# yifangao112/DinoUNet

Hardware: AMD Instinct MI355X
Metric: 2D slices/sec training, dinounet_l 512x512 bf16 (higher is better)
Workload: dtype bf16; 1 GPU; dinounet_l train step (fwd+loss+bwd+clip+SGD), 512x512x3 slices, batch 8/GPU, frozen ViT + adapter + FAPM + U-Net decoder, random-init weights; global_batch=8, parallelism=dp1

## Files before the change

dinounet_amd/_build.py:

```python
import hashlib
import os
import subprocess
import sys

HERE = os.path.dirname(os.path.abspath(__file__))
CSRC = os.path.join(HERE, "csrc")
LIB = os.path.join(HERE, "libdinounet_hip.so")
SOURCES = ["gemm.hip", "gemm_bf16.hip", "gemm_glds.hip", "gemm_p8.hip", "gemm_rk.hip", "gemm_skinny.hip", "conv_halo.hip", "conv_strip.hip", "attention.hip", "norm.hip", "msda.hip", "elementwise.hip", "loss.hip", "optim.hip", "augment.hip", "export.hip", "surface.hip"]
FLAGS = ["--offload-arch=gfx950", "-O3", "-std=c++17", "-fPIC", "-munsafe-fp-atomics", "-fno-gpu-rdc"]
if os.environ.get("DINOUNET_DEBUG_KNOBS") == "1":
    FLAGS.append("-DDU_DEBUG_KNOBS")
EXTRA_FLAGS = {"attention.hip": ["-mllvm", "-amdgpu-mfma-vgpr-form"], "conv_strip.hip": ["-mllvm", "-amdgpu-mfma-vgpr-form"]}
NO_SCRATCH = ("gemm_bf16.hip", "gemm_glds.hip", "gemm_p8.hip", "gemm_rk.hip", "gemm_skinny.hip", "conv_halo.hip", "conv_strip.hip", "attention.hip", "surface.hip")
REMARK = "-Rpass-analysis=kernel-resource-usage"
import re as _re
_ABLATION = _re.compile(
    r"attn_fwd_kernelILi\d+ELb1EEE"
    r"|attn_fwd_w64_kernelILi\d+ELi\d+ELb1E"
    r"|attn_fwd_w64_kernelILi\d+ELi\d+ELb\dELi\d+ELi[1-9]\d*ELi\d+EEE"
    r"|attn_fwd_pipe_kernelILb1ELi\d+EEE|attn_fwd_pipe_kernelILb\dELi[1-9]\d*EEE")


def _digest():
    h = hashlib.sha256()
    for f in sorted(os.listdir(CSRC)) + ["../../include/dinounet_hip.h"]:
        p = os.path.join(CSRC, f)
        if os.path.isfile(p):
            h.update(f.encode())
            h.update(open(p, "rb").read())
    h.update(" ".join(FLAGS).encode())
    h.update(repr(sorted(EXTRA_FLAGS.items())).encode())
    return h.hexdigest()


def build(force: bool = False, verbose: bool = True) -> str:
    stamp = LIB + ".stamp"
    dig = _digest()
    if not force and os.path.exists(LIB) and os.path.exists(stamp) and open(stamp).read() == dig:
        return LIB
    hipcc = os.environ.get("HIPCC", "/opt/rocm/bin/hipcc")
    objs, procs = [], []
    os.makedirs(os.path.join(HERE, "build"), exist_ok=True)
    for s in SOURCES:
        o = os.path.join(HERE, "build", s.replace(".hip", ".o"))
        objs.append(o)
        cmd = [hipcc, *FLAGS, *EXTRA_FLAGS.get(s, []), *([REMARK] if s in NO_SCRATCH else []), "-c", os.path.join(CSRC, s), "-o", o]
# ... 31 lines not shown
```

dinounet_amd/csrc/elementwise.hip:

```cpp
#include <stdlib.h>
#include "common.h"

namespace {

__host__ int grid_1d(long total) {
  long g = (total + 255) / 256;
  if (g < 1) g = 1;
  if (g > 65535L * 8) g = 65535L * 8;
  return (int)g;
}

#define GRID_STRIDE(i, total) for (long i = (long)blockIdx.x * 256 + threadIdx.x; i < (total); i += (long)gridDim.x * 256)

struct PyrPix { int b, s0, Hs, Ws, yo, xo; };
__device__ __forceinline__ PyrPix pyr_decode(long p, int H, int W) {
  const int n = (H * W) >> 2, N = 21 * n;
  PyrPix q;
  q.b = (int)(p / N);
  int t = (int)(p - (long)q.b * N);
  if (t < 16 * n) { q.s0 = 0; q.Hs = 2 * H; q.Ws = 2 * W; }
  else if (t < 20 * n) { q.s0 = 16 * n; q.Hs = H; q.Ws = W; t -= 16 * n; }
  else { q.s0 = 20 * n; q.Hs = H >> 1; q.Ws = W >> 1; t -= 20 * n; }
  q.yo = t / q.Ws; q.xo = t - q.yo * q.Ws;
  return q;
// ... 1065 lines not shown

extern "C" int du_patchify16(int dst_dtype, const float* src, void* dst, int B, int C, int H, int W, void* stream) {
  hipStream_t st = (hipStream_t)stream;
  if (!src || !dst || B <= 0 || H % 16 || W % 16) return DU_ERR_BAD_ARG;
  long total = (long)B * (H / 16) * (W / 16) * C * 256;
  DISPATCH_T(dst_dtype,
             hipLaunchKernelGGL(patchify16_kernel<bf16_t>, dim3(grid_1d(total)), dim3(256), 0, st, src, (bf16_t*)dst, B, C, H, W, total),
             hipLaunchKernelGGL(patchify16_kernel<float>, dim3(grid_1d(total)), dim3(256), 0, st, src, (float*)dst, B, C, H, W, total));
  return du_check_launch();
}

extern "C" int du_msda_prep(int dtype, const void* raw, int64_t ldr, const float* ref, float* loc, float* attn, int64_t rows, int Lq,
                            int M, int P, int Hs, int Ws, void* stream) {
  hipStream_t st = (hipStream_t)stream;
  if (!raw || !ref || !loc || !attn || rows <= 0 || Lq <= 0 || rows % Lq || M <= 0 || P <= 0 || P > 16) return DU_ERR_BAD_ARG;
  long total = rows * M;
  DISPATCH_T(dtype,
             hipLaunchKernelGGL(msda_prep_kernel<bf16_t>, dim3(grid_1d(total)), dim3(256), 0, st, (const bf16_t*)raw, ldr, ref, loc, attn, (long)rows, Lq, M, P, 1.f / Ws, 1.f / Hs, total),
             hipLaunchKernelGGL(msda_prep_kernel<float>, dim3(grid_1d(total)), dim3(256), 0, st, (const float*)raw, ldr, ref, loc, attn, (long)rows, Lq, M, P, 1.f / Ws, 1.f / Hs, total));
  return du_check_launch();
}

extern "C" int du_msda_prep_bwd(int dtype, const float* attn, const float* gloc, const float* gattn, void* graw, int64_t ldr, int64_t rows,
                                int M, int P, int Hs, int Ws, void* stream) {
  hipStream_t st = (hipStream_t)stream;
  if (!attn || !gloc || !gattn || !graw || rows <= 0 || M <= 0 || P <= 0) return DU_ERR_BAD_ARG;
  long total = rows * M;
  DISPATCH_T(dtype,
             hipLaunchKernelGGL(msda_prep_bwd_kernel<bf16_t>, dim3(grid_1d(total)), dim3(256), 0, st, attn, gloc, gattn, (bf16_t*)graw, ldr, (long)rows, M, P, 1.f / Ws, 1.f / Hs, total),
             hipLaunchKernelGGL(msda_prep_bwd_kernel<float>, dim3(grid_1d(total)), dim3(256), 0, st, attn, gloc, gattn, (float*)graw, ldr, (long)rows, M, P, 1.f / Ws, 1.f / Hs, total));
  return du_check_launch();
}

extern "C" int du_act_bwd(int dtype, const void* z, const void* dy, void* dz, int64_t n, int act, void* stream) {
  hipStream_t st = (hipStream_t)stream;
  if (!z || !dy || !dz || n <= 0) return DU_ERR_BAD_ARG;
  DISPATCH_T(dtype,
             hipLaunchKernelGGL(act_bwd_kernel<bf16_t>, dim3(grid_1d(n)), dim3(256), 0, st, (const bf16_t*)z, (const bf16_t*)dy, (bf16_t*)dz, (long)n, act),
             hipLaunchKernelGGL(act_bwd_kernel<float>, dim3(grid_1d(n)), dim3(256), 0, st, (const float*)z, (const float*)dy, (float*)dz, (long)n, act));
  return du_check_launch();
}

extern "C" int du_se_gate_fwd(const float* sums, float inv_count, const float* W1, const float* b1, const float* W2, const float* b2,
                              float* hidden, float* gate, int B, int C, int R, void* stream) {
  hipStream_t st = (hipStream_t)stream;
  if (!sums || !W1 || !b1 || !W2 || !b2 || !hidden || !gate || B <= 0 || C <= 0 || R <= 0) return DU_ERR_BAD_ARG;
  hipLaunchKernelGGL(se_gate_fwd_kernel, dim3(B), dim3(256), (C + R) * sizeof(float), st, sums, inv_count, W1, b1, W2, b2, hidden, gate, C, R);
  return du_check_launch();
}

extern "C" int du_se_scale_fwd(int dtype, const void* x, int64_t ldx, const float* gate, const void* shortcut, int64_t ldsc, void* y,
                               int64_t ldy, int B, int64_t P, int C, void* stream) {
  hipStream_t st = (hipStream_t)stream;
  const int v = dtype == DU_BF16 ? 8 : 4;
  if (!x || !gate || !y || B <= 0 || P <= 0 || C % v || ldx % v || ldy % v || (shortcut && ldsc % v)) return DU_ERR_BAD_ARG;
  long total = (long)B * P * (C / v);
  DISPATCH_T(dtype,
             hipLaunchKernelGGL(se_scale_kernel<bf16_t>, dim3(grid_1d(total)), dim3(256), 0, st, (const bf16_t*)x, ldx, gate, (const bf16_t*)shortcut, ldsc, (bf16_t*)y, ldy, (long)P, C, total),
             hipLaunchKernelGGL(se_scale_kernel<float>, dim3(grid_1d(total)), dim3(256), 0, st, (const float*)x, ldx, gate, (const float*)shortcut, ldsc, (float*)y, ldy, (long)P, C, total));
  return du_check_launch();
}

extern "C" int du_se_gate_bwd(const float* dsum, const float* sums, float inv_count, const float* gate, const float* hidden,
                              const float* W1, const float* W2, float* dpool, float* dW1, float* db1, float* dW2, float* db2, int B, int C,
                              int R, void* stream) {
  hipStream_t st = (hipStream_t)stream;
  if (!dsum || !sums || !gate || !hidden || !W1 || !W2 || !dpool || !dW1 || !db1 || !dW2 || !db2 || B <= 0 || C <= 0 || R <= 0)
    return DU_ERR_BAD_ARG;
  int Bc = (int)(8000 / (long)(C + R));
  if (Bc < 1) return DU_ERR_UNSUPPORTED;
  if (Bc > B) Bc = B;
  hipLaunchKernelGGL(se_gate_bwd_kernel, dim3(1), dim3(1024), (size_t)2 * Bc * (C + R) * sizeof(float), st, dsum, sums, inv_count, gate, hidden,
// ... 339 lines not shown
```

dinounet_amd/csrc/gemm_p8.hip:

```cpp
#include <algorithm>
#include <vector>
#include "common.h"
#include "gemm_params.h"
#include "gemm_plan.h"
#include "gemm_skinny_body.h"

namespace {

typedef __attribute__((address_space(3))) void lds_void;

constexpr int PBM = 256, PBN = 256, PBK = 64;
constexpr int HALF_B = 128 * PBK * 2;
constexpr int BUF_B = 4 * HALF_B;
constexpr int STG_LD = PBN + 4;

template <typename TC> struct Out4p;
template <> struct Out4p<float> {
  static __device__ __forceinline__ void load(const float* p, float* v) { float4 t = *(const float4*)p; v[0] = t.x; v[1] = t.y; v[2] = t.z; v[3] = t.w; }
  static __device__ __forceinline__ void store(float* p, const float* v) { *(float4*)p = make_float4(v[0], v[1], v[2], v[3]); }
};
template <> struct Out4p<bf16_t> {
  static __device__ __forceinline__ void load(const bf16_t* p, float* v) {
    bf16x4 t = __builtin_bit_cast(bf16x4, *(const uint2*)p);
#pragma unroll
// ... 2020 lines not shown
    attr_set[g_p8_sched ? 1 : 0] = true;
  }
  hipLaunchKernelGGL(kfn, grid, dim3(512), P8_LDS, st, P);
  return du_check_launch();
}

int g_p8_tn = 1;

template <int SCHED, bool GA>
int launch_p8_tn(const du_gemm_args& a, int splits, hipStream_t st) {
  GemmParams P = make_params(a, DU_PLAIN_COL, GA ? DU_IM2COL_COL : DU_PLAIN_COL, PBM, PBN, PBK);
  P.tiles_m = (a.M + PBM - 1) / PBM;
  P.split_k = splits;
  P.k_per_split = 0;
  P.dbg = g_p8_debug;
  dim3 grid(P.tiles_m * P.tiles_n * splits, 1);
  void (*kfn)(GemmParams) = GA ? gemm_nt_p8_kernel<float, SCHED, true, true> : gemm_nt_p8_kernel<float, SCHED, true, false>;
  static bool attr_set = false;
  if (!attr_set) {
    if (hipFuncSetAttribute((const void*)kfn, hipFuncAttributeMaxDynamicSharedMemorySize, P8_LDS) != hipSuccess) return DU_ERR_LAUNCH;
    attr_set = true;
  }
  hipLaunchKernelGGL(kfn, grid, dim3(512), P8_LDS, st, P);
  return du_check_launch();
}

}

extern int g_attn_w;
extern int g_attn_impl, g_attn_thresh_log2, g_attn_var;
extern int g_rk_mode;
extern int g_wgrad_rows;
extern int g_ln_rows2;

extern "C" int du_set_option(int key, int value) {
  switch (key) {
    case 4: g_attn_w = value; return DU_OK;
    case 6: g_attn_impl = value; return DU_OK;
    case 7: g_attn_thresh_log2 = value; return DU_OK;
    case 8: g_attn_var = value; return DU_OK;
    case 0: g_p8_mode = value; return DU_OK;
    case 1: g_p8_sched = value; return DU_OK;
    case 2: g_p8_group = value; return DU_OK;
    case 3: g_p8_debug = value; return DU_OK;
    case 5: g_p8_tn = value; return DU_OK;
    case 9: g_p8_corun = value < 1 ? 1 : (value > 8 ? 8 : value); return DU_OK;
    case 10: g_p8_persist = value; return DU_OK;
    case 11: g_p8_pp_full = value; return DU_OK;
    case 12: g_rk_mode = value; return DU_OK;
    case 13: g_wgrad_rows = value; return DU_OK;
    case 14: g_p8_res = value; return DU_OK;
    case 15: g_p8_tail_inline = value; return DU_OK;
    case 16: g_p8_ks = value; return DU_OK;
    case 17: g_p8_tail_slices = value; return DU_OK;
    case 18: g_ln_rows2 = value; return DU_OK;
    default: return DU_ERR_BAD_ARG;
  }
}

static bool convt_gather_geom(const du_gemm_args& a, const void* src, long ld, long pixels_in) {
  const du_conv_geom& g = a.geom;
  if (g.KH != 2 || g.KW != 2 || g.stride != 2 || g.pad != 0 || g.transposed || g.p2) return false;
  if (g.Hi != 2 * g.Ho || g.Wi != 2 * g.Wo || g.Ho <= 0 || g.Wo <= 0) return false;
  if (g.C <= 0 || (g.C & (g.C - 1)) || g.C % 64 || ld % 8 || (((uintptr_t)src) & 15)) return false;
  if (pixels_in % ((long)g.Ho * g.Wo)) return false;
  return 4 * pixels_in * ld * 2 <= 0x7fffffffL;
}
static bool p8_gather_legal(const du_gemm_args& a) {
  if (a.a_mode != DU_IM2COL_ROW || a.b_mode != DU_PLAIN_ROW || a.dtype != DU_BF16 || a.out_dtype != DU_BF16) return false;
  if (a.split_k > 1 || a.batch > 1 || a.store_mode != DU_STORE_PLAIN || a.act == DU_ACT_SWIGLU) return false;
  if (!convt_gather_geom(a, a.A, a.lda, a.M) || a.K != 4 * a.geom.C) return false;
  if (a.K % 128 || a.M < 256 || a.N < 128 || a.N % 4 || a.ldb % 8 || (((uintptr_t)a.B) & 15)) return false;
  return (long)a.ldb * 2 * 256 <= 0x7fffffffL;
}

bool p8_legal(const du_gemm_args& a) {
  if (a.a_mode != DU_PLAIN_ROW || a.b_mode != DU_PLAIN_ROW || a.dtype != DU_BF16) return false;
  if (a.split_k > 1) return false;
  if (a.store_mode == DU_STORE_MSDA_PREP) {
    if (a.out_dtype != DU_F32 || a.residual || a.gamma || a.row_scale || a.alpha != 1.0f || a.act != DU_ACT_NONE || a.batch > 1) return false;
    if (a.N % 12 || a.N > 256 || a.ps_H <= 0 || a.ps_W <= 0 || a.ps_C <= 0 || !a.rope_sin || !a.C2) return false;
    if ((((uintptr_t)a.C) | ((uintptr_t)a.C2)) & 15) return false;
  } else
  if (a.store_mode == DU_STORE_QKV_ROPE || a.store_mode == DU_STORE_QKV_HEADS) {
    if (a.out_dtype != DU_BF16 || a.residual || a.gamma || a.row_scale || a.alpha != 1.0f || a.act != DU_ACT_NONE || a.batch > 1) return false;
    if (a.ps_H <= 0 || a.ps_W < a.ps_H || a.ps_C <= 0 || a.N != 3 * a.ps_C * 64 || a.ldc % 8 || (((uintptr_t)a.C) & 15)) return false;
    if (a.store_mode == DU_STORE_QKV_ROPE && (!a.rope_sin || !a.rope_cos || ((((uintptr_t)a.rope_sin) | ((uintptr_t)a.rope_cos)) & 15))) return false;
  } else
// ... 242 lines not shown
```

dinounet_amd/ops.py:

```python
import ctypes as C
import math
import os
import weakref

import torch

from . import _lib
from ._lib import (ACT_GELU, ACT_LEAKY, ACT_NONE, ACT_RELU, ACT_SWIGLU, DU_BF16, DU_F32, IM2COL_COL, IM2COL_ROW, PLAIN_COL,
                   PLAIN_ROW, STORE_MSDA_PREP, STORE_PIXEL_SHUFFLE2, STORE_QKV_HEADS, STORE_QKV_ROPE, STORE_SLABS, ConvGeom, GemmArgs)

__all__ = ["mm", "linear", "conv2d", "conv_transpose2x2", "norm_act", "layer_norm", "msda", "dwconv3x3",
           "maxpool3x3s2", "bilinear_add", "bilinear_resize", "squeeze_excite", "dice_ce_loss", "dice_ce_masked_loss", "dice_bce_loss",
           "labels_to_regions", "val_dice_ce", "val_dice_bce"]


def _code(dt):
    if dt == torch.bfloat16:
        return DU_BF16
    if dt == torch.float32:
        return DU_F32
    raise RuntimeError(f"dinounet_amd: unsupported dtype {dt} (bf16 / fp32 only)")


def _req(*ts):
# ... 1713 lines not shown
        ctx.lc_saved = None
        ctx.save_for_backward(xs, wq, attn)
        ctx.prep = (M, P, Hs, Ws, ncol)
        return loc, attn

    @staticmethod
    def backward(ctx, gloc, gattn):
        x, wq, attn = ctx.saved_tensors
        M, P, Hs, Ws, ncol = ctx.prep
        rows = attn.shape[0]
        graw = torch.empty((rows, ncol), dtype=x.dtype, device=attn.device)
        _lib.check(_lib.lib().du_msda_prep_bwd(_code(x.dtype), _p(attn), _p(gloc.contiguous()), _p(gattn.contiguous()), _p(graw), ncol, rows,
                                               M, P, Hs, Ws, _st()), "du_msda_prep_bwd")
        return (*_linear_cat_bwd(ctx, graw, x, wq), None, None, None, None, None, None)


def offsets_prep(x, w1, w2, b1, b2, ref, Lq, M, P, Hs, Ws):
    return _OffsetsPrep.apply(x.reshape(-1, x.shape[-1]), w1, w2, b1, b2, ref, Lq, M, P, Hs, Ws)


class _DWConvSegs(torch.autograd.Function):

    @staticmethod
    def forward(ctx, x, w, bias, segs, act):
        x = x.contiguous()
        Cc = w.shape[0]
        wf = _f32(w).view(Cc, 9)
        bf = _f32(bias)
        y = torch.empty_like(x)
        z = torch.empty_like(x) if act != ACT_NONE else None
        es = x.element_size()
        L = _lib.lib()
        for (off, B, h, ww, ld, bs) in segs:
            _lib.check(L.du_dwconv3x3_fwd(_code(x.dtype), C.c_void_p(x.data_ptr() + off * es), ld, bs, _p(wf), _p(bf),
                                          C.c_void_p(y.data_ptr() + off * es), ld, bs,
                                          None if z is None else C.c_void_p(z.data_ptr() + off * es), B, h, ww, Cc, act, _st()),
                       "du_dwconv3x3_fwd")
        ctx.save_for_backward(x, wf, z)
        ctx.conf = (segs, act, bias is not None, Cc)
        return y

    @staticmethod
    def backward(ctx, dy):
        x, wf, z = ctx.saved_tensors
        segs, act, has_bias, Cc = ctx.conf
        L = _lib.lib()
        es = x.element_size()
        code = _code(x.dtype)
        dy = dy.contiguous()
        if act != ACT_NONE:
            dz = torch.empty_like(dy)
            _lib.check(L.du_act_bwd(code, _p(z), _p(dy), _p(dz), dy.numel(), act, _st()), "du_act_bwd")
        else:
            dz = dy
        dx = torch.empty_like(x)
        dw = torch.empty((Cc, 9), dtype=torch.float32, device=x.device)
        db = torch.empty(Cc, dtype=torch.float32, device=x.device) if has_bias else None
        for si, (off, B, h, ww, ld, bs) in enumerate(segs):
            _lib.check(L.du_dwconv3x3_bwd_data(code, C.c_void_p(dz.data_ptr() + off * es), ld, bs, _p(wf),
                                               C.c_void_p(dx.data_ptr() + off * es), ld, bs, B, h, ww, Cc, _st()),
                       "du_dwconv3x3_bwd_data")
            n = int(L.du_dwconv_wgrad_ws_elems(code, B, h, ww, Cc))
            ws = torch.empty(max(n, 1), dtype=torch.float32, device=x.device)
            _lib.check(L.du_dwconv3x3_bwd_weight(code, C.c_void_p(x.data_ptr() + off * es), ld, bs,
                                                 C.c_void_p(dz.data_ptr() + off * es), ld, bs, _p(dw), _p(db), B, h, ww, Cc,
                                                 _p(ws), n, 1 if si > 0 else 0, _st()), "du_dwconv3x3_bwd_weight")
        return dx, dw.view(Cc, 1, 3, 3), db, None, None


def dwconv3x3(x, w, bias=None, act=ACT_NONE):
    x = x.contiguous()
    B, H, W, Cc = x.shape
    return _DWConvSegs.apply(x, w, bias, ((0, B, H, W, Cc, H * W * Cc),), act)


class _DWConvTokens(torch.autograd.Function):

    @staticmethod
    def forward(ctx, x, w, bias, H, W, act):
        x = x.contiguous()
        B, N, Cc = x.shape
        wf = _f32(w).view(Cc, 9)
        y = torch.empty_like(x)
        z = torch.empty_like(x) if act != ACT_NONE else None
        _lib.check(_lib.lib().du_dwconv3x3_tokens_fwd(_code(x.dtype), _p(x), _p(wf), _p(_f32(bias)), _p(y), _p(z), B, H, W, Cc, act, _st()),
                   "du_dwconv3x3_tokens_fwd")
        ctx.save_for_backward(x, wf, z)
        ctx.conf = (H, W, act, bias is not None)
        return y

    @staticmethod
    def backward(ctx, dy):
        x, wf, z = ctx.saved_tensors
        H, W, act, has_bias = ctx.conf
        B, N, Cc = x.shape
        L = _lib.lib()
        code = _code(x.dtype)
        dy = dy.contiguous()
        if act != ACT_NONE:
            dz = torch.empty_like(dy)
            _lib.check(L.du_act_bwd(code, _p(z), _p(dy), _p(dz), dy.numel(), act, _st()), "du_act_bwd")
        else:
            dz = dy
        dx = torch.empty_like(x)
        _lib.check(L.du_dwconv3x3_tokens_bwd_data(code, _p(dz), _p(wf), _p(dx), B, H, W, Cc, _st()), "du_dwconv3x3_tokens_bwd_data")
        dw = torch.empty((Cc, 9), dtype=torch.float32, device=x.device)
        db = torch.empty(Cc, dtype=torch.float32, device=x.device) if has_bias else None
        n = int(L.du_dwconv_wgrad_ws_elems(code, B, N, 1, Cc))
        ws = torch.empty(max(n, 1), dtype=torch.float32, device=x.device)
        _lib.check(L.du_dwconv3x3_tokens_bwd_weight(code, _p(x), _p(dz), _p(dw), _p(db), B, H, W, Cc, _p(ws), n, _st()),
                   "du_dwconv3x3_tokens_bwd_weight")
        return dx, dw.view(Cc, 1, 3, 3), db, None, None, None


def dwconv_tokens(x, w, bias, H, W, act=ACT_GELU):
    B, N, Cc = x.shape
    assert N == 21 * ((H * W) // 4) and H % 2 == 0 and W % 2 == 0, (N, H, W)
    return _DWConvTokens.apply(x, w, bias, H, W, act)


class _MaxPool(torch.autograd.Function):
    @staticmethod
    def forward(ctx, x):
        x = x.contiguous()
        B, H, W, Cc = x.shape
        Ho, Wo = (H - 1) // 2 + 1, (W - 1) // 2 + 1
        y = torch.empty((B, Ho, Wo, Cc), dtype=x.dtype, device=x.device)
        idx = torch.empty((B, Ho, Wo, Cc), dtype=torch.uint8, device=x.device)
        _lib.check(_lib.lib().du_maxpool3x3s2_fwd(_code(x.dtype), _p(x), _p(y), _p(idx), B, H, W, Cc, _st()), "du_maxpool3x3s2_fwd")
        ctx.save_for_backward(idx)
        ctx.shape = (B, H, W, Cc, x.dtype)
# ... 533 lines not shown
```

include/dinounet_hip.h:

```cpp
#ifndef DINOUNET_HIP_H
#define DINOUNET_HIP_H

#include <stdint.h>

#ifdef __cplusplus
extern "C" {
#endif

#define DU_OK 0
#define DU_ERR_BAD_ARG (-1)
#define DU_ERR_UNSUPPORTED (-2)
#define DU_ERR_LAUNCH (-3)

#define DU_F32 0
#define DU_BF16 1

#define DU_PLAIN_ROW 0
#define DU_PLAIN_COL 1
#define DU_IM2COL_ROW 2
#define DU_IM2COL_COL 3

#define DU_ACT_NONE 0
#define DU_ACT_GELU 1
#define DU_ACT_RELU 2
// ... 125 lines not shown
                     const float* sampling_loc, const float* attn_weight, const void* grad_out, float* grad_value,
                     float* grad_sampling_loc, float* grad_attn_weight, int N, int S, int M, int D, int L, int Lq, int P,
                     float* ws, int64_t ws_elems, void* stream);

int du_msda_forward_f64(const double* value, const int64_t* spatial_shapes, const int64_t* level_start_index, const double* sampling_loc,
                        const double* attn_weight, double* out, int N, int S, int M, int D, int L, int Lq, int P, void* stream);
int du_msda_backward_f64(const double* value, const int64_t* spatial_shapes, const int64_t* level_start_index, const double* sampling_loc,
                         const double* attn_weight, const double* grad_out, double* grad_value, double* grad_sampling_loc,
                         double* grad_attn_weight, int N, int S, int M, int D, int L, int Lq, int P, void* stream);

int du_msda_backward_bf16gv(const void* value, const int64_t* spatial_shapes, const int64_t* level_start_index, const float* sampling_loc,
                            const float* attn_weight, const void* grad_out, void* grad_value_bf16, float* grad_sampling_loc,
                            float* grad_attn_weight, int N, int S, int M, int D, int L, int Lq, int P, float* ws, int64_t ws_elems,
                            void* stream);

int du_msda_prep(int dtype, const void* raw, int64_t ldr, const float* ref, float* loc, float* attn, int64_t rows, int Lq,
                 int M, int P, int Hs, int Ws, void* stream);
int du_msda_prep_bwd(int dtype, const float* attn, const float* gloc, const float* gattn, void* graw, int64_t ldr,
                     int64_t rows, int M, int P, int Hs, int Ws, void* stream);

int du_dwconv3x3_fwd(int dtype, const void* x, int64_t ldx, int64_t xbs, const float* w, const float* bias, void* y,
                     int64_t ldy, int64_t ybs, void* z, int B, int H, int W, int C, int act, void* stream);
int du_dwconv3x3_bwd_data(int dtype, const void* dy, int64_t lddy, int64_t dybs, const float* w, void* dx, int64_t lddx,
                          int64_t dxbs, int B, int H, int W, int C, void* stream);
int64_t du_dwconv_wgrad_ws_elems(int dtype, int B, int H, int W, int C);
int du_dwconv3x3_bwd_weight(int dtype, const void* x, int64_t ldx, int64_t xbs, const void* dy, int64_t lddy, int64_t dybs,
                            float* dw, float* db, int B, int H, int W, int C, float* ws, int64_t ws_elems, int accumulate,
                            void* stream);
int du_dwconv3x3_tokens_fwd(int dtype, const void* x, const float* w, const float* bias, void* y, void* z, int B, int H, int W, int C,
                            int act, void* stream);
int du_dwconv3x3_tokens_bwd_data(int dtype, const void* dy, const float* w, void* dx, int B, int H, int W, int C, void* stream);
int du_dwconv3x3_tokens_bwd_weight(int dtype, const void* x, const void* dy, float* dw, float* db, int B, int H, int W, int C, float* ws,
                                   int64_t ws_elems, void* stream);
int du_maxpool3x3s2_fwd(int dtype, const void* x, void* y, uint8_t* idx, int B, int H, int W, int C, void* stream);
int du_maxpool3x3s2_bwd(int dtype, const uint8_t* idx, const void* dy, void* dx, int B, int H, int W, int C, void* stream);
int du_bilinear_add_fwd(int src_dtype, int dtype, const void* src, int64_t lds_, const void* base, int64_t ldb, void* out,
                        int64_t ldo, int B, int Hs, int Ws, int Ho, int Wo, int C, void* stream);
int du_bilinear_resize_bwd(int dtype, const void* dy, int64_t lddy, void* dx, int64_t lddx, int B, int Hs, int Ws, int Ho, int Wo,
                           int C, void* stream);
int du_act_bwd(int dtype, const void* z, const void* dy, void* dz, int64_t n, int act, void* stream);

int du_se_gate_fwd(const float* sums, float inv_count, const float* W1, const float* b1, const float* W2, const float* b2,
                   float* hidden, float* gate, int B, int C, int R, void* stream);
int du_se_scale_fwd(int dtype, const void* x, int64_t ldx, const float* gate, const void* shortcut, int64_t ldsc, void* y, int64_t ldy,
                    int B, int64_t P, int C, void* stream);
int du_se_gate_bwd(const float* dsum, const float* sums, float inv_count, const float* gate, const float* hidden, const float* W1,
                   const float* W2, float* dpool, float* dW1, float* db1, float* dW2, float* db2, int B, int C, int R, void* stream);
int du_se_scale_bwd(int dtype, const void* dy, int64_t lddy, const float* gate, const float* dpool, void* dx, int64_t lddx, int B,
                    int64_t P, int C, void* stream);

int64_t du_dice_ce_ws_elems(int B, int K, int64_t HW);
int du_dice_ce_sums(const float* logits, const int64_t* target, float* sums, int B, int K, int64_t HW, float* ws, int64_t ws_elems,
                    void* stream);
int du_dice_ce_finish(const float* sums, float* loss, float* coef, int K, int64_t npix, float smooth, float grad_mult, void* stream);
int du_dice_ce_bwd(const float* logits, const int64_t* target, const float* coef, const float* grad_out, float* dlogits, int B, int K,
                   int64_t HW, void* stream);

int64_t du_dice_ce_masked_ws_elems(int B, int K, int64_t HW);
int du_dice_ce_masked_sums(const float* logits, const int64_t* target, float* sums, int B, int K, int64_t HW, int64_t ignore_label,
                           float* ws, int64_t ws_elems, void* stream);
int du_dice_ce_masked_finish(const float* sums, float* loss, float* coef, int K, float smooth, float grad_mult, void* stream);
int du_dice_ce_masked_bwd(const float* logits, const int64_t* target, const float* coef, const float* grad_out, float* dlogits, int B,
                          int K, int64_t HW, int64_t ignore_label, void* stream);

int64_t du_dice_bce_ws_elems(int B, int R, int64_t HW);
int du_dice_bce_sums(const float* logits, const uint8_t* target, float* sums, int B, int R, int64_t HW, int has_ignore, float* ws,
// ... 84 lines not shown
```

Baseline: 305.2 slices/s.

## Add row-band register-streaming depthwise 3x3 conv kernels with fused act-grad backward

Adds a new dwconv.hip with band-tiled depthwise 3x3 kernels. Each thread streams rows of an 8-channel by 2-column tile through registers, reusing the three-row window instead of reloading neighbours. The backward pass fuses the activation gradient into data-grad, sharing tile edges through shared memory, and computes weight-grad as per-block partials plus a finalize reduction. Workgroups are ordered XCD-aware, and band height is picked by a simple cost model. It also caps the act_bwd grid size, at the cost of more code paths and a workspace allocation per backward call.

```diff
diff --git a/dinounet_amd/_build.py b/dinounet_amd/_build.py
--- a/dinounet_amd/_build.py
+++ b/dinounet_amd/_build.py
@@ -6,12 +6,12 @@
 HERE = os.path.dirname(os.path.abspath(__file__))
 CSRC = os.path.join(HERE, "csrc")
 LIB = os.path.join(HERE, "libdinounet_hip.so")
-SOURCES = ["gemm.hip", "gemm_bf16.hip", "gemm_glds.hip", "gemm_p8.hip", "gemm_rk.hip", "gemm_skinny.hip", "conv_halo.hip", "conv_strip.hip", "attention.hip", "norm.hip", "msda.hip", "elementwise.hip", "loss.hip", "optim.hip", "augment.hip", "export.hip", "surface.hip"]
+SOURCES = ["gemm.hip", "gemm_bf16.hip", "gemm_glds.hip", "gemm_p8.hip", "gemm_rk.hip", "gemm_skinny.hip", "conv_halo.hip", "conv_strip.hip", "attention.hip", "norm.hip", "msda.hip", "elementwise.hip", "dwconv.hip", "loss.hip", "optim.hip", "augment.hip", "export.hip", "surface.hip"]
 FLAGS = ["--offload-arch=gfx950", "-O3", "-std=c++17", "-fPIC", "-munsafe-fp-atomics", "-fno-gpu-rdc"]
 if os.environ.get("DINOUNET_DEBUG_KNOBS") == "1":
     FLAGS.append("-DDU_DEBUG_KNOBS")
 EXTRA_FLAGS = {"attention.hip": ["-mllvm", "-amdgpu-mfma-vgpr-form"], "conv_strip.hip": ["-mllvm", "-amdgpu-mfma-vgpr-form"]}
-NO_SCRATCH = ("gemm_bf16.hip", "gemm_glds.hip", "gemm_p8.hip", "gemm_rk.hip", "gemm_skinny.hip", "conv_halo.hip", "conv_strip.hip", "attention.hip", "surface.hip")
+NO_SCRATCH = ("gemm_bf16.hip", "gemm_glds.hip", "gemm_p8.hip", "gemm_rk.hip", "gemm_skinny.hip", "conv_halo.hip", "conv_strip.hip", "attention.hip", "surface.hip", "dwconv.hip")
 REMARK = "-Rpass-analysis=kernel-resource-usage"
 import re as _re
 _ABLATION = _re.compile(
diff --git a/dinounet_amd/csrc/dwconv.hip b/dinounet_amd/csrc/dwconv.hip
--- /dev/null
+++ b/dinounet_amd/csrc/dwconv.hip
@@ -0,0 +1,485 @@
+#include "common.h"
+
+int g_dwconv_band = 1;
+
+namespace {
+
+constexpr int XT = 2;
+constexpr int CVB = 8;
+constexpr int NL = 32;
+constexpr int V = 8;
+
+struct BandGeom {
+  long ld, bs;
+  int C, R, nlev, nslab;
+  int Hs[3], Ws[3], s0[3];
+  int ncg[3], nbands[3], nitems[3], nblk[3];
+  int wg0[4];
+  int row0[3];
+};
+
+__device__ __forceinline__ int xcd_linear_index() {
+  const int nwg = gridDim.x, bid = blockIdx.x;
+  const int q = nwg >> 3, r = nwg & 7, xcd = bid & 7, idx = bid >> 3;
+  return (xcd < r ? xcd * (q + 1) : r * (q + 1) + (xcd - r) * q) + idx;
+}
+
+#define LEV(a, l) ((l) == 0 ? (a)[0] : ((l) == 1 ? (a)[1] : (a)[2]))
+
+struct Item {
+  bool on;
+  int y0, y1, x0, Hs, Ws, cg, ncg, c0, prow, slab;
+  long base;
+};
+
+__device__ __forceinline__ Item band_item(const BandGeom& G) {
+  const int lin = xcd_linear_index();
+  int l = 0;
+  if (G.nlev > 1 && lin >= G.wg0[1]) l = 1;
+  if (G.nlev > 2 && lin >= G.wg0[2]) l = 2;
+  const int nblk = LEV(G.nblk, l), r = lin - LEV(G.wg0, l);
+  const int slab = r / nblk, blk = r - slab * nblk;
+  const int lane = threadIdx.x / CVB, tcv = threadIdx.x % CVB;
+  const int item = blk * NL + lane, cv = slab * CVB + tcv;
+  Item it;
+  it.ncg = LEV(G.ncg, l);
+  it.Hs = LEV(G.Hs, l);
+  it.Ws = LEV(G.Ws, l);
+  it.prow = LEV(G.row0, l) + blk;
+  it.slab = slab;
+  it.on = item < LEV(G.nitems, l) && cv * V < G.C;
+  const int nb = LEV(G.nbands, l);
+  const int t = item / it.ncg, b = t / nb, band = t - b * nb;
+  it.cg = item - t * it.ncg;
+  it.x0 = it.cg * XT;
+  it.y0 = it.on ? band * G.R : 0;
+  it.y1 = it.on ? min(it.Hs, it.y0 + G.R) : 0;
+  it.c0 = cv * V;
+  it.base = it.on ? (long)b * G.bs + (long)LEV(G.s0, l) * G.ld + it.c0 : 0;
+  return it;
+}
+
+struct Row { uint4 c[XT + 2]; };
+
+__device__ __forceinline__ Row zero_row() {
+  Row r;
+#pragma unroll
+  for (int c = 0; c < XT + 2; c++) r.c[c] = make_uint4(0, 0, 0, 0);
+  return r;
+}
+
+__device__ __forceinline__ Row load_row(const bf16_t* __restrict__ p, const Item& it, long ld, int yi, bool want) {
+  Row r;
+  const bool rv = want && yi >= 0 && yi < it.Hs;
+  const bf16_t* row = p + it.base + (long)yi * it.Ws * ld;
+#pragma unroll
+  for (int c = 0; c < XT + 2; c++) {
+    const int xi = it.x0 - 1 + c;
+    r.c[c] = (rv && xi >= 0 && xi < it.Ws) ? *(const uint4*)(row + (long)xi * ld) : make_uint4(0, 0, 0, 0);
+  }
+  return r;
+}
+
+__device__ __forceinline__ void load_taps(const float* __restrict__ w, const float* __restrict__ bias, int c0, bool flip, float (&wt)[9][V],
+                                          float (&bs)[V]) {
+#pragma unroll
+  for (int j = 0; j < V; j++) {
+    bs[j] = bias ? bias[c0 + j] : 0.f;
+#pragma unroll
+    for (int t = 0; t < 9; t++) wt[t][j] = w[(c0 + j) * 9 + (flip ? 8 - t : t)];
+  }
+}
+
+__device__ __forceinline__ void stencil(const Row& a, const Row& b, const Row& c, const float (&wt)[9][V], const float (&bs)[V],
+                                        float (&acc)[XT][V]) {
+#pragma unroll
+  for (int t = 0; t < XT; t++)
+#pragma unroll
+    for (int j = 0; j < V; j++) acc[t][j] = bs[j];
+#pragma unroll
+  for (int dy = 0; dy < 3; dy++) {
+    const Row& r = dy == 0 ? a : (dy == 1 ? b : c);
+#pragma unroll
+    for (int cc = 0; cc < XT + 2; cc++) {
+      const Vec16<bf16_t> v = as_vec<bf16_t>(r.c[cc]);
+      float f[V];
+#pragma unroll
+      for (int j = 0; j < V; j++) f[j] = to_f32(v.v[j]);
+#pragma unroll
+      for (int dx = 0; dx < 3; dx++) {
+        const int t = cc - dx;
+        if (t >= 0 && t < XT) {
+#pragma unroll
+          for (int j = 0; j < V; j++) acc[t][j] += f[j] * wt[dy * 3 + dx][j];
+        }
+      }
+    }
+  }
+}
+
+template <bool FLIP, int ACT>
+__global__ __launch_bounds__(256) void dwconv_band_kernel(const bf16_t* __restrict__ x, const float* __restrict__ w,
+                                                          const float* __restrict__ bias, bf16_t* __restrict__ y, bf16_t* __restrict__ z,
+                                                          BandGeom G, int act_rt) {
+  const int act = ACT >= 0 ? ACT : act_rt;
+  const Item it = band_item(G);
+  if (!it.on) return;
+  float wt[9][V], bs[V];
+  load_taps(w, bias, it.c0, FLIP, wt, bs);
+  Row a = load_row(x, it, G.ld, it.y0 - 1, true), b = load_row(x, it, G.ld, it.y0, true), c = load_row(x, it, G.ld, it.y0 + 1, true);
+  for (int yo = it.y0; yo < it.y1; yo++) {
+    const Row n = load_row(x, it, G.ld, yo + 2, yo + 2 <= it.y1);
+    float acc[XT][V];
+    stencil(a, b, c, wt, bs, acc);
+    const long off = it.base + ((long)yo * it.Ws + it.x0) * G.ld;
+#pragma unroll
+    for (int t = 0; t < XT; t++) {
+      Vec16<bf16_t> o;
+      if (!FLIP && z) {
+#pragma unroll
+        for (int j = 0; j < V; j++) o.v[j] = from_f32<bf16_t>(acc[t][j]);
+        *(uint4*)(z + off + (long)t * G.ld) = as_u4(o);
+      }
+#pragma unroll
+      for (int j = 0; j < V; j++) o.v[j] = from_f32<bf16_t>(FLIP ? acc[t][j] : apply_act(acc[t][j], act));
+      *(uint4*)(y + off + (long)t * G.ld) = as_u4(o);
+    }
+    a = b; b = c; c = n;
+  }
+}
+
+__device__ __forceinline__ uint4 act_dz(uint4 zr, uint4 gr, int act) {
+  const Vec16<bf16_t> a = as_vec<bf16_t>(zr), g = as_vec<bf16_t>(gr);
+  Vec16<bf16_t> o;
+#pragma unroll
+  for (int j = 0; j < V; j++) o.v[j] = from_f32<bf16_t>(to_f32(g.v[j]) * act_grad(to_f32(a.v[j]), act));
+  return as_u4(o);
+}
+
+template <int ACT, bool SELF>
+__global__ __launch_bounds__(256) void dwconv_band_dgrad_act_kernel(const bf16_t* __restrict__ z, const bf16_t* __restrict__ dy,
+                                                                    const float* __restrict__ w, bf16_t* __restrict__ dx,
+                                                                    bf16_t* __restrict__ dzo, BandGeom G, int act_rt) {
+  __shared__ uint4 edge[2][256][2];
+  const int act = ACT >= 0 ? ACT : act_rt;
+  const Item it = band_item(G);
+  const int tid = threadIdx.x, lane = tid / CVB;
+  float wt[9][V], bs[V];
+  if (it.on) load_taps(w, nullptr, it.c0, true, wt, bs);
+  else {
+#pragma unroll
+    for (int j = 0; j < V; j++) {
+      bs[j] = 0.f;
+#pragma unroll
+      for (int t = 0; t < 9; t++) wt[t][j] = 0.f;
+    }
+  }
+  const bool lz = it.cg == 0, rz = it.cg == it.ncg - 1;
+  const bool lself = SELF && !lz && lane == 0, rself = SELF && !rz && lane == NL - 1;
+  Row a = zero_row(), b = zero_row(), c = zero_row();
+  uint4 zc[XT], gc[XT];
+  {
+    const int yi = it.y0 - 1;
+    const bool rv = it.on && yi >= 0;
+    const long off = it.base + ((long)yi * it.Ws + it.x0) * G.ld;
+#pragma unroll
+    for (int t = 0; t < XT; t++) {
+      zc[t] = rv ? *(const uint4*)(z + off + (long)t * G.ld) : make_uint4(0, 0, 0, 0);
+      gc[t] = rv ? *(const uint4*)(dy + off + (long)t * G.ld) : make_uint4(0, 0, 0, 0);
+    }
+  }
+  for (int i = 0; i < G.R + 2; i++) {
+    const int yi = it.y0 - 1 + i, p = i & 1;
+    const bool rv = it.on && yi >= 0 && yi < it.Hs && yi <= it.y1;
+    uint4 zn[XT], gn[XT];
+    {
+      const bool nv = it.on && yi + 1 < it.Hs && yi + 1 <= it.y1;
+      const long off = it.base + ((long)(yi + 1) * it.Ws + it.x0) * G.ld;
+#pragma unroll
+      for (int t = 0; t < XT; t++) {
+        zn[t] = nv ? *(const uint4*)(z + off + (long)t * G.ld) : make_uint4(0, 0, 0, 0);
+        gn[t] = nv ? *(const uint4*)(dy + off + (long)t * G.ld) : make_uint4(0, 0, 0, 0);
+      }
+    }
+    Row n;
+    const long roff = it.base + ((long)yi * it.Ws + it.x0) * G.ld;
+#pragma unroll
+    for (int t = 0; t < XT; t++) n.c[1 + t] = rv ? act_dz(zc[t], gc[t], act) : make_uint4(0, 0, 0, 0);
+    if (rv && yi >= it.y0 && yi < it.y1) {
+#pragma unroll
+      for (int t = 0; t < XT; t++) *(uint4*)(dzo + roff + (long)t * G.ld) = n.c[1 + t];
+    }
+    edge[p][tid][0] = n.c[1];
+    edge[p][tid][1] = n.c[XT];
+    __syncthreads();
+    n.c[0] = make_uint4(0, 0, 0, 0);
+    n.c[XT + 1] = make_uint4(0, 0, 0, 0);
+    if (rv) {
+      if (lself) n.c[0] = act_dz(*(const uint4*)(z + roff - G.ld), *(const uint4*)(dy + roff - G.ld), act);
+      else if (!lz) n.c[0] = edge[p][tid - CVB][1];
+      if (rself) n.c[XT + 1] = act_dz(*(const uint4*)(z + roff + (long)XT * G.ld), *(const uint4*)(dy + roff + (long)XT * G.ld), act);
+      else if (!rz) n.c[XT + 1] = edge[p][tid + CVB][0];
+    }
+    a = b; b = c; c = n;
+    const int yo = yi - 1;
+    if (i >= 2 && it.on && yo < it.y1) {
+      float acc[XT][V];
+      stencil(a, b, c, wt, bs, acc);
+      const long off = it.base + ((long)yo * it.Ws + it.x0) * G.ld;
+#pragma unroll
+      for (int t = 0; t < XT; t++) {
+        Vec16<bf16_t> o;
+#pragma unroll
+        for (int j = 0; j < V; j++) o.v[j] = from_f32<bf16_t>(acc[t][j]);
+        *(uint4*)(dx + off + (long)t * G.ld) = as_u4(o);
+      }
+    }
+#pragma unroll
+    for (int t = 0; t < XT; t++) { zc[t] = zn[t]; gc[t] = gn[t]; }
+  }
+}
+
+__global__ __launch_bounds__(256) void dwconv_band_wgrad_kernel(const bf16_t* __restrict__ x, const bf16_t* __restrict__ dz,
+                                                                float* __restrict__ part, BandGeom G) {
+  __shared__ float red[5][256 * V];
+  const Item it = band_item(G);
+  float aw[10][V];
+#pragma unroll
+  for (int k = 0; k < 10; k++)
+#pragma unroll
+    for (int j = 0; j < V; j++) aw[k][j] = 0.f;
+  if (it.on) {
+    Row a = load_row(x, it, G.ld, it.y0 - 1, true), b = load_row(x, it, G.ld, it.y0, true), c = load_row(x, it, G.ld, it.y0 + 1, true);
+    uint4 gc[XT];
+#pragma unroll
+    for (int t = 0; t < XT; t++) gc[t] = *(const uint4*)(dz + it.base + ((long)it.y0 * it.Ws + it.x0 + t) * G.ld);
+    for (int yo = it.y0; yo < it.y1; yo++) {
+      const Row n = load_row(x, it, G.ld, yo + 2, yo + 2 <= it.y1);
+      uint4 gn[XT];
+#pragma unroll
+      for (int t = 0; t < XT; t++)
+        gn[t] = yo + 1 < it.y1 ? *(const uint4*)(dz + it.base + ((long)(yo + 1) * it.Ws + it.x0 + t) * G.ld) : make_uint4(0, 0, 0, 0);
+      float gf[XT][V];
+#pragma unroll
+      for (int t = 0; t < XT; t++) {
+        const Vec16<bf16_t> g = as_vec<bf16_t>(gc[t]);
+#pragma unroll
+        for (int j = 0; j < V; j++) { gf[t][j] = to_f32(g.v[j]); aw[9][j] += gf[t][j]; }
+      }
+#pragma unroll
+      for (int ky = 0; ky < 3; ky++) {
+        const Row& r = ky == 0 ? a : (ky == 1 ? b : c);
+#pragma unroll
+        for (int cc = 0; cc < XT + 2; cc++) {
+          const Vec16<bf16_t> v = as_vec<bf16_t>(r.c[cc]);
+          float f[V];
+#pragma unroll
+          for (int j = 0; j < V; j++) f[j] = to_f32(v.v[j]);
+#pragma unroll
+          for (int kx = 0; kx < 3; kx++) {
+            const int t = cc - kx;
+            if (t >= 0 && t < XT) {
+#pragma unroll
+              for (int j = 0; j < V; j++) aw[ky * 3 + kx][j] += f[j] * gf[t][j];
+            }
+          }
+        }
+      }
+      a = b; b = c; c = n;
+#pragma unroll
+      for (int t = 0; t < XT; t++) gc[t] = gn[t];
+    }
+  }
+  const int slab = it.slab;
+  constexpr int NCOL = CVB * V;
+#pragma unroll
+  for (int half = 0; half < 2; half++) {
+#pragma unroll
+    for (int k = 0; k < 5; k++)
+#pragma unroll
+      for (int j = 0; j < V; j++) red[k][threadIdx.x * V + j] = aw[half * 5 + k][j];
+    __syncthreads();
+    for (int o = threadIdx.x; o < 5 * NCOL; o += 256) {
+      const int k5 = o / NCOL, ci = o - k5 * NCOL;
+      const int ch = slab * NCOL + ci;
+      if (ch >= G.C) continue;
+      float s0 = 0.f, s1 = 0.f, s2 = 0.f, s3 = 0.f;
+#pragma unroll
+      for (int q = 0; q < NL; q += 4) {
+        s0 += red[k5][q * NCOL + ci];
+        s1 += red[k5][(q + 1) * NCOL + ci];
+        s2 += red[k5][(q + 2) * NCOL + ci];
+        s3 += red[k5][(q + 3) * NCOL + ci];
+      }
+      part[((long)it.prow * 10 + half * 5 + k5) * G.C + ch] = (s0 + s1) + (s2 + s3);
+    }
+    __syncthreads();
+  }
+}
+
+__global__ __launch_bounds__(256) void dwconv_band_finalize_kernel(const float* __restrict__ part, float* __restrict__ dw,
+                                                                   float* __restrict__ db, int rows, int C, int accum) {
+  __shared__ float red[8][33];
+  const int col = threadIdx.x & 31, sl = threadIdx.x >> 5;
+  const int i = blockIdx.x * 32 + col, n = C * 10;
+  float s0 = 0.f, s1 = 0.f, s2 = 0.f, s3 = 0.f;
+  if (i < n) {
+    int r = sl;
+    for (; r + 24 < rows; r += 32) {
+      s0 += part[(long)r * n + i];
+      s1 += part[(long)(r + 8) * n + i];
+      s2 += part[(long)(r + 16) * n + i];
+      s3 += part[(long)(r + 24) * n + i];
+    }
+    for (; r < rows; r += 8) s0 += part[(long)r * n + i];
+  }
+  red[sl][col] = (s0 + s1) + (s2 + s3);
+  __syncthreads();
+  if (sl == 0 && i < n) {
+    float t = 0.f;
+#pragma unroll
+    for (int q = 0; q < 8; q++) t += red[q][col];
+    const int k = i / C, c = i - k * C;
+    if (k < 9) dw[c * 9 + k] = accum ? dw[c * 9 + k] + t : t;
+    else if (db) db[c] = accum ? db[c] + t : t;
+  }
+}
+
+bool band_shape_ok(int dtype, int B, int H, int W, int C, int pyramid) {
+  if (!g_dwconv_band || dtype != DU_BF16 || B <= 0 || H <= 0 || W <= 0 || C <= 0 || C % V) return false;
+  if (pyramid) {
+    if ((H & 1) || (W & 1) || (W / 2) % XT) return false;
+    if ((long)B * 21 * ((long)H * W / 4) * ((C + 63) / 64) > 0x3fffffffL) return false;
+  } else {
+    if (W % XT) return false;
+    if ((long)B * H * W * ((C + 63) / 64) > 0x3fffffffL) return false;
+  }
+  return true;
+}
+
+void band_count(BandGeom& G, int B) {
+  int wg = 0, row = 0;
+  for (int l = 0; l < G.nlev; l++) {
+    G.ncg[l] = G.Ws[l] / XT;
+    G.nbands[l] = (G.Hs[l] + G.R - 1) / G.R;
+    G.nitems[l] = B * G.nbands[l] * G.ncg[l];
+    G.nblk[l] = (G.nitems[l] + NL - 1) / NL;
+    G.wg0[l] = wg; G.row0[l] = row;
+    wg += G.nblk[l] * G.nslab; row += G.nblk[l];
+  }
+  G.wg0[G.nlev] = wg;
+}
+
+int band_rows(const BandGeom& G) { return G.row0[G.nlev - 1] + G.nblk[G.nlev - 1]; }
+
+BandGeom band_geom(int B, int H, int W, int C, int pyramid, long ld, long bs, int rows_cap) {
+  BandGeom G{};
+  G.ld = ld; G.bs = bs; G.C = C;
+  G.nslab = (C + CVB * V - 1) / (CVB * V);
+  if (pyramid) {
+    const int n = (H * W) >> 2;
+    G.nlev = 3;
+    G.Hs[0] = 2 * H; G.Ws[0] = 2 * W; G.s0[0] = 0;
+    G.Hs[1] = H; G.Ws[1] = W; G.s0[1] = 16 * n;
+    G.Hs[2] = H >> 1; G.Ws[2] = W >> 1; G.s0[2] = 20 * n;
+  } else {
+    G.nlev = 1;
+    G.Hs[0] = H; G.Ws[0] = W; G.s0[0] = 0;
+  }
+  const int forced = rows_cap > 0 ? (g_dwconv_band >> 8) & 0xff : (g_dwconv_band >= 2 ? g_dwconv_band & 0xff : 0);
+  if (forced >= 2) G.R = forced;
+  else {
+    const int slots = 512;
+    long best = 0;
+    int pick = 4;
+    for (int r = 4; r <= 16; r++) {
+      G.R = r;
+      band_count(G, B);
+      const long cost = (long)((G.wg0[G.nlev] + slots - 1) / slots) * (2 * r + 3);
+      if (r == 4 || cost < best) { best = cost; pick = r; }
+    }
+    G.R = pick;
+  }
+  for (;;) {
+    band_count(G, B);
+    if (rows_cap <= 0 || band_rows(G) <= rows_cap || G.R >= G.Hs[0]) break;
+    G.R *= 2;
+  }
+  return G;
+}
+
+constexpr int WGRAD_ROWS_CAP = 512;
+
+void band_forward(const bf16_t* x, const float* w, const float* bias, bf16_t* y, bf16_t* z, const BandGeom& G, int act, hipStream_t st) {
+  const dim3 grid(G.wg0[G.nlev]), block(256);
+  if (act == DU_ACT_GELU) hipLaunchKernelGGL((dwconv_band_kernel<false, DU_ACT_GELU>), grid, block, 0, st, x, w, bias, y, z, G, act);
+  else if (act == DU_ACT_NONE) hipLaunchKernelGGL((dwconv_band_kernel<false, DU_ACT_NONE>), grid, block, 0, st, x, w, bias, y, z, G, act);
+  else hipLaunchKernelGGL((dwconv_band_kernel<false, -1>), grid, block, 0, st, x, w, bias, y, z, G, act);
+}
+
+int band_backward(const bf16_t* z, const bf16_t* dy, const bf16_t* x, const float* w, bf16_t* dx, float* dw, float* db, bf16_t* dz, int B,
+                  int H, int W, int C, int pyramid, long ld, long bs, int act, float* ws, int64_t ws_elems, int accumulate, hipStream_t st) {
+  const BandGeom G = band_geom(B, H, W, C, pyramid, ld, bs, 0);
+  const bf16_t* g = dy;
+  if (act != DU_ACT_NONE) {
+    if (!z || !dz) return DU_ERR_BAD_ARG;
+    bool cut = false;
+    for (int l = 0; l < G.nlev; l++) cut = cut || NL % G.ncg[l] != 0;
+    const dim3 grid(G.wg0[G.nlev]), block(256);
+    if (act == DU_ACT_GELU && !cut) hipLaunchKernelGGL((dwconv_band_dgrad_act_kernel<DU_ACT_GELU, false>), grid, block, 0, st, z, dy, w, dx, dz, G, act);
+    else if (act == DU_ACT_GELU) hipLaunchKernelGGL((dwconv_band_dgrad_act_kernel<DU_ACT_GELU, true>), grid, block, 0, st, z, dy, w, dx, dz, G, act);
+    else hipLaunchKernelGGL((dwconv_band_dgrad_act_kernel<-1, true>), grid, block, 0, st, z, dy, w, dx, dz, G, act);
+    g = dz;
+  } else {
+    hipLaunchKernelGGL((dwconv_band_kernel<true, DU_ACT_NONE>), dim3(G.wg0[G.nlev]), dim3(256), 0, st, dy, w, (const float*)nullptr, dx,
+                       (bf16_t*)nullptr, G, (int)DU_ACT_NONE);
+  }
+  const BandGeom GW = band_geom(B, H, W, C, pyramid, ld, bs, WGRAD_ROWS_CAP);
+  const int rows = band_rows(GW);
+  if (!ws || ws_elems < (int64_t)rows * 10 * C) return DU_ERR_BAD_ARG;
+  hipLaunchKernelGGL(dwconv_band_wgrad_kernel, dim3(GW.wg0[GW.nlev]), dim3(256), 0, st, x, g, ws, GW);
+  hipLaunchKernelGGL(dwconv_band_finalize_kernel, dim3((C * 10 + 31) / 32), dim3(256), 0, st, (const float*)ws, dw, db, rows, C, accumulate);
+  return du_check_launch();
+}
+
+}
+
+extern "C" int du_dwconv_band_ok(int dtype, int B, int H, int W, int C, int pyramid) { return band_shape_ok(dtype, B, H, W, C, pyramid) ? 1 : 0; }
+
+extern "C" int64_t du_dwconv_band_ws_elems(int dtype, int B, int H, int W, int C, int pyramid) {
+  if (!band_shape_ok(dtype, B, H, W, C, pyramid)) return 0;
+  return (int64_t)band_rows(band_geom(B, H, W, C, pyramid, C, 0, WGRAD_ROWS_CAP)) * 10 * C;
+}
+
+extern "C" int du_dwconv_band_tokens_fwd(int dtype, const void* x, const float* w, const float* bias, void* y, void* z, int B, int H, int W,
+                                         int C, int act, void* stream) {
+  if (!x || !w || !y || !band_shape_ok(dtype, B, H, W, C, 1)) return DU_ERR_BAD_ARG;
+  const long N = 21L * ((H * W) >> 2);
+  const BandGeom G = band_geom(B, H, W, C, 1, C, N * C, 0);
+  band_forward((const bf16_t*)x, w, bias, (bf16_t*)y, (bf16_t*)z, G, act, (hipStream_t)stream);
+  return du_check_launch();
+}
+
+extern "C" int du_dwconv_band_tokens_bwd(int dtype, const void* z, const void* dy, const void* x, const float* w, void* dx, float* dw,
+                                         float* db, void* dz, int B, int H, int W, int C, int act, float* ws, int64_t ws_elems,
+                                         void* stream) {
+  if (!dy || !x || !w || !dx || !dw || !band_shape_ok(dtype, B, H, W, C, 1)) return DU_ERR_BAD_ARG;
+  const long N = 21L * ((H * W) >> 2);
+  return band_backward((const bf16_t*)z, (const bf16_t*)dy, (const bf16_t*)x, w, (bf16_t*)dx, dw, db, (bf16_t*)dz, B, H, W, C, 1, C, N * C, act,
+                       ws, ws_elems, 0, (hipStream_t)stream);
+}
+
+extern "C" int du_dwconv_band_fwd(int dtype, const void* x, const float* w, const float* bias, void* y, int64_t ld, int64_t bs, int B, int H,
+                                  int W, int C, void* stream) {
+  if (!x || !w || !y || ld % V || bs % V || !band_shape_ok(dtype, B, H, W, C, 0)) return DU_ERR_BAD_ARG;
+  const BandGeom G = band_geom(B, H, W, C, 0, ld, bs, 0);
+  band_forward((const bf16_t*)x, w, bias, (bf16_t*)y, (bf16_t*)nullptr, G, DU_ACT_NONE, (hipStream_t)stream);
+  return du_check_launch();
+}
+
+extern "C" int du_dwconv_band_bwd(int dtype, const void* dy, const void* x, const float* w, void* dx, float* dw, float* db, int64_t ld,
+                                  int64_t bs, int B, int H, int W, int C, float* ws, int64_t ws_elems, int accumulate, void* stream) {
+  if (!dy || !x || !w || !dx || !dw || ld % V || bs % V || !band_shape_ok(dtype, B, H, W, C, 0)) return DU_ERR_BAD_ARG;
+  return band_backward(nullptr, (const bf16_t*)dy, (const bf16_t*)x, w, (bf16_t*)dx, dw, db, nullptr, B, H, W, C, 0, ld, bs, DU_ACT_NONE, ws,
+                       ws_elems, accumulate, (hipStream_t)stream);
+}
diff --git a/dinounet_amd/csrc/elementwise.hip b/dinounet_amd/csrc/elementwise.hip
--- a/dinounet_amd/csrc/elementwise.hip
+++ b/dinounet_amd/csrc/elementwise.hip
@@ -1121,12 +1121,17 @@
   return du_check_launch();
 }
 
+static inline int act_bwd_grid(long n, int v) {
+  const long g = (n / v + 255) / 256;
+  return (int)(g < 1 ? 1 : (g > 2048 ? 2048 : g));
+}
+
 extern "C" int du_act_bwd(int dtype, const void* z, const void* dy, void* dz, int64_t n, int act, void* stream) {
   hipStream_t st = (hipStream_t)stream;
   if (!z || !dy || !dz || n <= 0) return DU_ERR_BAD_ARG;
   DISPATCH_T(dtype,
-             hipLaunchKernelGGL(act_bwd_kernel<bf16_t>, dim3(grid_1d(n)), dim3(256), 0, st, (const bf16_t*)z, (const bf16_t*)dy, (bf16_t*)dz, (long)n, act),
-             hipLaunchKernelGGL(act_bwd_kernel<float>, dim3(grid_1d(n)), dim3(256), 0, st, (const float*)z, (const float*)dy, (float*)dz, (long)n, act));
+             hipLaunchKernelGGL(act_bwd_kernel<bf16_t>, dim3(act_bwd_grid(n, 8)), dim3(256), 0, st, (const bf16_t*)z, (const bf16_t*)dy, (bf16_t*)dz, (long)n, act),
+             hipLaunchKernelGGL(act_bwd_kernel<float>, dim3(act_bwd_grid(n, 4)), dim3(256), 0, st, (const float*)z, (const float*)dy, (float*)dz, (long)n, act));
   return du_check_launch();
 }
 
diff --git a/dinounet_amd/csrc/gemm_p8.hip b/dinounet_amd/csrc/gemm_p8.hip
--- a/dinounet_amd/csrc/gemm_p8.hip
+++ b/dinounet_amd/csrc/gemm_p8.hip
@@ -2076,6 +2076,7 @@
 extern int g_rk_mode;
 extern int g_wgrad_rows;
 extern int g_ln_rows2;
+extern int g_dwconv_band;
 
 extern "C" int du_set_option(int key, int value) {
   switch (key) {
@@ -2098,6 +2099,7 @@
     case 16: g_p8_ks = value; return DU_OK;
     case 17: g_p8_tail_slices = value; return DU_OK;
     case 18: g_ln_rows2 = value; return DU_OK;
+    case 19: g_dwconv_band = value < 0 ? 0 : value; return DU_OK;
     default: return DU_ERR_BAD_ARG;
   }
 }
diff --git a/dinounet_amd/ops.py b/dinounet_amd/ops.py
--- a/dinounet_amd/ops.py
+++ b/dinounet_amd/ops.py
@@ -1769,6 +1769,10 @@
         es = x.element_size()
         L = _lib.lib()
         for (off, B, h, ww, ld, bs) in segs:
+            if act == ACT_NONE and L.du_dwconv_band_ok(_code(x.dtype), B, h, ww, Cc, 0):
+                _lib.check(L.du_dwconv_band_fwd(_code(x.dtype), C.c_void_p(x.data_ptr() + off * es), _p(wf), _p(bf),
+                                                C.c_void_p(y.data_ptr() + off * es), ld, bs, B, h, ww, Cc, _st()), "du_dwconv_band_fwd")
+                continue
             _lib.check(L.du_dwconv3x3_fwd(_code(x.dtype), C.c_void_p(x.data_ptr() + off * es), ld, bs, _p(wf), _p(bf),
                                           C.c_void_p(y.data_ptr() + off * es), ld, bs,
                                           None if z is None else C.c_void_p(z.data_ptr() + off * es), B, h, ww, Cc, act, _st()),
@@ -1794,6 +1798,13 @@
         dw = torch.empty((Cc, 9), dtype=torch.float32, device=x.device)
         db = torch.empty(Cc, dtype=torch.float32, device=x.device) if has_bias else None
         for si, (off, B, h, ww, ld, bs) in enumerate(segs):
+            if act == ACT_NONE and L.du_dwconv_band_ok(code, B, h, ww, Cc, 0):
+                n = int(L.du_dwconv_band_ws_elems(code, B, h, ww, Cc, 0))
+                ws = torch.empty(max(n, 1), dtype=torch.float32, device=x.device)
+                _lib.check(L.du_dwconv_band_bwd(code, C.c_void_p(dz.data_ptr() + off * es), C.c_void_p(x.data_ptr() + off * es), _p(wf),
+                                                C.c_void_p(dx.data_ptr() + off * es), _p(dw), _p(db), ld, bs, B, h, ww, Cc, _p(ws), n,
+                                                1 if si > 0 else 0, _st()), "du_dwconv_band_bwd")
+                continue
             _lib.check(L.du_dwconv3x3_bwd_data(code, C.c_void_p(dz.data_ptr() + off * es), ld, bs, _p(wf),
                                                C.c_void_p(dx.data_ptr() + off * es), ld, bs, B, h, ww, Cc, _st()),
                        "du_dwconv3x3_bwd_data")
@@ -1820,8 +1831,13 @@
         wf = _f32(w).view(Cc, 9)
         y = torch.empty_like(x)
         z = torch.empty_like(x) if act != ACT_NONE else None
-        _lib.check(_lib.lib().du_dwconv3x3_tokens_fwd(_code(x.dtype), _p(x), _p(wf), _p(_f32(bias)), _p(y), _p(z), B, H, W, Cc, act, _st()),
-                   "du_dwconv3x3_tokens_fwd")
+        L = _lib.lib()
+        if L.du_dwconv_band_ok(_code(x.dtype), B, H, W, Cc, 1):
+            _lib.check(L.du_dwconv_band_tokens_fwd(_code(x.dtype), _p(x), _p(wf), _p(_f32(bias)), _p(y), _p(z), B, H, W, Cc, act, _st()),
+                       "du_dwconv_band_tokens_fwd")
+        else:
+            _lib.check(L.du_dwconv3x3_tokens_fwd(_code(x.dtype), _p(x), _p(wf), _p(_f32(bias)), _p(y), _p(z), B, H, W, Cc, act, _st()),
+                       "du_dwconv3x3_tokens_fwd")
         ctx.save_for_backward(x, wf, z)
         ctx.conf = (H, W, act, bias is not None)
         return y
@@ -1834,6 +1850,16 @@
         L = _lib.lib()
         code = _code(x.dtype)
         dy = dy.contiguous()
+        if L.du_dwconv_band_ok(code, B, H, W, Cc, 1):
+            dz = torch.empty_like(dy) if act != ACT_NONE else None
+            dx = torch.empty_like(x)
+            dw = torch.empty((Cc, 9), dtype=torch.float32, device=x.device)
+            db = torch.empty(Cc, dtype=torch.float32, device=x.device) if has_bias else None
+            n = int(L.du_dwconv_band_ws_elems(code, B, H, W, Cc, 1))
+            ws = torch.empty(max(n, 1), dtype=torch.float32, device=x.device)
+            _lib.check(L.du_dwconv_band_tokens_bwd(code, _p(z), _p(dy), _p(x), _p(wf), _p(dx), _p(dw), _p(db), _p(dz), B, H, W, Cc, act,
+                                                   _p(ws), n, _st()), "du_dwconv_band_tokens_bwd")
+            return dx, dw.view(Cc, 1, 3, 3), db, None, None, None
         if act != ACT_NONE:
             dz = torch.empty_like(dy)
             _lib.check(L.du_act_bwd(code, _p(z), _p(dy), _p(dz), dy.numel(), act, _st()), "du_act_bwd")
diff --git a/include/dinounet_hip.h b/include/dinounet_hip.h
--- a/include/dinounet_hip.h
+++ b/include/dinounet_hip.h
@@ -181,6 +181,16 @@
 int du_dwconv3x3_tokens_bwd_data(int dtype, const void* dy, const float* w, void* dx, int B, int H, int W, int C, void* stream);
 int du_dwconv3x3_tokens_bwd_weight(int dtype, const void* x, const void* dy, float* dw, float* db, int B, int H, int W, int C, float* ws,
                                    int64_t ws_elems, void* stream);
+int du_dwconv_band_ok(int dtype, int B, int H, int W, int C, int pyramid);
+int64_t du_dwconv_band_ws_elems(int dtype, int B, int H, int W, int C, int pyramid);
+int du_dwconv_band_tokens_fwd(int dtype, const void* x, const float* w, const float* bias, void* y, void* z, int B, int H, int W, int C,
+                              int act, void* stream);
+int du_dwconv_band_tokens_bwd(int dtype, const void* z, const void* dy, const void* x, const float* w, void* dx, float* dw, float* db,
+                              void* dz, int B, int H, int W, int C, int act, float* ws, int64_t ws_elems, void* stream);
+int du_dwconv_band_fwd(int dtype, const void* x, const float* w, const float* bias, void* y, int64_t ld, int64_t bs, int B, int H, int W,
+                       int C, void* stream);
+int du_dwconv_band_bwd(int dtype, const void* dy, const void* x, const float* w, void* dx, float* dw, float* db, int64_t ld, int64_t bs,
+                       int B, int H, int W, int C, float* ws, int64_t ws_elems, int accumulate, void* stream);
 int du_maxpool3x3s2_fwd(int dtype, const void* x, void* y, uint8_t* idx, int B, int H, int W, int C, void* stream);
 int du_maxpool3x3s2_bwd(int dtype, const uint8_t* idx, const void* dy, void* dx, int B, int H, int W, int C, void* stream);
 int du_bilinear_add_fwd(int src_dtype, int dtype, const void* src, int64_t lds_, const void* base, int64_t ldb, void* out,
```

Measured after the change: 310.0 slices/s (median of 6 runs). 1.02x the previous value.
